# wangzy22/UniPre3D

Hardware: AMD Instinct MI355X
Metric: rendered_views_per_sec (higher is better)
Workload: dtype f32; 1 GPU; C2: render-loss hot path (activations + render fwd + loss + render bwd), object-level, P=128 Gaussians/object, 256x256, B=32/GPU x V=4 views = 128 renders/GPU/step; head output o ~ N(0,1) i.i.d. (SURVEY 8d primary regime); global_batch=32, parallelism=dp1, loss=focal_l2, autograd_entry=loss.backward()

## Files before the change

__graft_entry__.py:

```python
import os
import subprocess
import sys

ROOT = os.path.dirname(os.path.abspath(__file__))
if ROOT not in sys.path:
    sys.path.insert(0, ROOT)


def build() -> None:
    res = subprocess.run(["make", "-C", os.path.join(ROOT, "unipre3d_amd", "csrc"), "-j4"], capture_output=True, text=True)
    if res.returncode != 0:
        raise RuntimeError("HIP build failed:\n" + res.stdout[-3000:] + res.stderr[-3000:])
    import shutil
    csrc, var = os.path.join(ROOT, "unipre3d_amd", "csrc"), os.path.join(ROOT, "unipre3d_amd", "lib_general")
    res = subprocess.run(["make", "-C", csrc, "-j4", "LIBDIR=../lib_general", "EXTRA=-DU3D_FORCE_GENERAL", "../lib_general/libunipre3d_rasterizer.so"],
                         capture_output=True, text=True)
    if res.returncode != 0:
        raise RuntimeError("HIP build (test variant) failed:\n" + res.stdout[-3000:] + res.stderr[-3000:])
    shutil.copy2(os.path.join(ROOT, "unipre3d_amd", "lib", "_u3d_torch.so"), os.path.join(var, "_u3d_torch.so"))
    res = subprocess.run(["make", "-C", os.path.join(ROOT, "oracle")], capture_output=True, text=True)
    if res.returncode != 0:
        raise RuntimeError("oracle build failed:\n" + res.stdout[-3000:] + res.stderr[-3000:])
    import unipre3d_amd
    from unipre3d_amd import _lib
    lib = _lib.load()
    for name in _lib.EXPORTS:
        getattr(lib, name)
    from unipre3d_amd import rasterizer
    binding = rasterizer._C()
    for name in ("rasterize_view", "rasterize_batched", "render_loss_step", "unit_tensor", "abi_version"):
        getattr(binding, name)
    from unipre3d_amd import pointops
    po = pointops.load()
    for name in pointops.EXPORTS:
# ... 81 lines not shown
```

unipre3d_amd/csrc/u3d_common.h:

```cpp
#pragma once
#include <hip/hip_runtime.h>
#include <stdint.h>

#include "unipre3d_rasterizer.h"

#define U3D_TILE 16
#define U3D_BLOCK 256
#define U3D_WAVE 64
#define U3D_FLAG_INTERNAL_TRIAGE 0x40000000
#define U3D_TOUCHED_BIT 0x80000000u
#define U3D_TILE_PLAIN_BIT 0x80000000u
#define U3D_NACC 10
#define U3D_LDS_SORT_MAX 4096
static_assert(U3D_LDS_SORT_MAX == U3D_SPARSE_BWD_MIN_P, "the public header's sparse-backward threshold is this limit (the torch binding sizes its buffers by it)");
#ifndef U3D_RADIX_NT_SMALL
#define U3D_RADIX_NT_SMALL 1024
#define U3D_RADIX_IT_SMALL 2
#define U3D_RADIX_NT_LARGE 1024
#define U3D_RADIX_IT_LARGE 4
#endif
static inline int u3d_radix_tile(int P) { return P <= 65536 ? U3D_RADIX_NT_SMALL * U3D_RADIX_IT_SMALL : U3D_RADIX_NT_LARGE * U3D_RADIX_IT_LARGE; }
#define U3D_MSD_BINS_MAX 2048
static inline int u3d_msd_bins(int P) { return P <= 65536 ? 512 : (P <= 262144 ? 1024 : 2048); }
#define U3D_MSD_KEY_BASE 0x3E4CCCCDu

struct U3DBuffers {
  float* depth;
  float2* xy;
  float4* conic_op;
  float4* rgbd;
  uint2* rect;
  uint32_t* clamped;
  uint32_t* num_rendered;
  uint32_t* touched_words;
  uint2* touched_list;
  uint32_t* touched_count;
  uint32_t* sorted_id;
  uint2* sorted_rect;
  uint32_t* n_vis;
  uint32_t* sort_keys[2];
  uint32_t* sort_vals[2];
  uint2* sort_pairs;
  uint32_t* sort_hist;
  uint32_t* sort_over;
  float* final_T;
  uint32_t* n_contrib;
  uint32_t* tile_last;
};

struct U3DSpan {
  const int32_t* off;
  int P, vpi;
};
static inline U3DSpan u3d_span(const u3d_raster_desc& d) { return U3DSpan{d.total_P > 0 ? d.item_offsets : nullptr, d.P, d.views_per_item}; }
// ... 71 lines not shown
  float* qnorm; float* qdot; float* partial;
};
static inline size_t u3d_carve_fused(const u3d_raster_desc& d, void* base, U3DFused* f) {
  const size_t NV = (size_t)d.n_items * d.views_per_item;
  const size_t T = (size_t)((d.image_width + U3D_TILE - 1) / U3D_TILE) * ((d.image_height + U3D_TILE - 1) / U3D_TILE);
  const size_t a = (((size_t)d.n_items * 4 * sizeof(float)) + 255) & ~(size_t)255;
  if (f) {
    f->qnorm = (float*)base;
    f->qdot = (float*)((char*)base + a);
    f->partial = (float*)((char*)base + 2 * a);
  }
  return 2 * a + (((NV * T * sizeof(float)) + 255) & ~(size_t)255) + 256;
}

#define U3D_PART_BLOCKS 2
static inline int u3d_part_blocks(const u3d_raster_desc& d) { return d.P <= 256 ? 1 : U3D_PART_BLOCKS; }
#define U3D_PART_STRIDE (U3D_PART_BLOCKS * U3D_WAVE * 10)
static inline size_t u3d_align(size_t x) { return (x + 255) & ~(size_t)255; }

static inline U3DLayout u3d_carve(const u3d_raster_desc& d, void* geom, void* binning, void* image, U3DBuffers* b) {
  const size_t NV = (size_t)d.n_items * d.views_per_item, NG = (size_t)d.views_per_item * u3d_total_P(d);
  const size_t NP = NV * (size_t)d.image_height * d.image_width;
  U3DLayout L{};
  size_t o = 0;
  char* g = (char*)geom;
#define CARVE(base, field, type, count)        \
  do {                                         \
    if (b) b->field = (type*)(base + o);       \
    o += u3d_align(sizeof(type) * (count));    \
  } while (0)
  CARVE(g, depth, float, NG);
  CARVE(g, xy, float2, NG);
  CARVE(g, conic_op, float4, NG);
// ... 12 lines not shown
  CARVE(bn, sorted_rect, uint2, NG);
  CARVE(bn, n_vis, uint32_t, NV);
  if (d.P > U3D_LDS_SORT_MAX) {
    CARVE(bn, sort_keys[0], uint32_t, NG);
    CARVE(bn, sort_keys[1], uint32_t, NG);
    CARVE(bn, sort_vals[0], uint32_t, NG);
    CARVE(bn, sort_vals[1], uint32_t, NG);
    CARVE(bn, sort_pairs, uint2, NG);
    const size_t nblk = ((size_t)d.P + u3d_radix_tile(d.P) - 1) / u3d_radix_tile(d.P);
    CARVE(bn, sort_hist, uint32_t, NV * (size_t)u3d_msd_bins(d.P) * (nblk + 1));
    CARVE(bn, sort_over, uint32_t, NV * ((size_t)u3d_msd_bins(d.P) + 1));
  } else if (b) {
    b->sort_keys[0] = b->sort_keys[1] = b->sort_vals[0] = b->sort_vals[1] = b->sort_hist = b->sort_over = nullptr;
    b->sort_pairs = nullptr;
  }
  L.binning_bytes = o > 0 ? o : 256;
  o = 0;
  char* im = (char*)image;
  CARVE(im, final_T, float, NP);
  CARVE(im, n_contrib, uint32_t, NP);
  CARVE(im, tile_last, uint32_t, NV * (size_t)((d.image_width + U3D_TILE - 1) / U3D_TILE) * ((d.image_height + U3D_TILE - 1) / U3D_TILE));
  L.image_bytes = o > 0 ? o : 256;
#undef CARVE
  L.acc_bytes = u3d_align(sizeof(double) * U3D_NACC * (NG > 0 ? NG : 1));
  {
    const size_t Tn = (size_t)((d.image_width + U3D_TILE - 1) / U3D_TILE) * ((d.image_height + U3D_TILE - 1) / U3D_TILE);
    L.backward_bytes = L.acc_bytes + u3d_align(sizeof(float) * U3D_PART_STRIDE * (NV * Tn > 0 ? NV * Tn : 1)) +
                       u3d_align(sizeof(uint32_t) * (NV * Tn > 0 ? NV * Tn : 1));
  }
  L.fused_bytes = u3d_carve_fused(d, nullptr, nullptr);
// ... 107 lines not shown
```

unipre3d_amd/csrc/u3d_preprocess.hip:

```cpp
#include "u3d_common.h"

#pragma clang fp contract(off)

namespace {

constexpr float SH_C0 = 0.28209479177387814f;
constexpr float SH_C1 = 0.4886025119029199f;
__device__ constexpr float SH_C2[5] = {1.0925484305920792f, -1.0925484305920792f, 0.31539156525252005f,
                                       -1.0925484305920792f, 0.5462742152960396f};
__device__ constexpr float SH_C3[7] = {-0.5900435899266435f, 2.890611442640554f, -0.4570457994644658f,
                                       0.3731763325901154f,  -0.4570457994644658f, 1.445305721320277f,
                                       -0.5900435899266435f};

struct Cam {
  float V[16], Pm[16], pos[3];
};

__device__ __forceinline__ void load_cam(Cam& c, const float* __restrict__ view, const float* __restrict__ proj,
                                         const float* __restrict__ campos, int v) {
#pragma unroll
  for (int k = 0; k < 16; ++k) { c.V[k] = view[v * 16 + k]; c.Pm[k] = proj[v * 16 + k]; }
#pragma unroll
  for (int k = 0; k < 3; ++k) c.pos[k] = campos[v * 3 + k];
}
// ... 81 lines not shown
    for (int k = 0; k < 4; ++k) {
      g.raw_q[k] = g.q[k];
      g.qn[k] = fmaxf(src.act == 1 ? src.qnorm[item * 4 + k] : n4, 1e-6f);
      g.q[k] = g.q[k] / g.qn[k];
    }
  }
}

template <int D>
__global__ __launch_bounds__(U3D_BLOCK) void preprocess_fwd_kernel(
    U3DSpan span, int vpi, int vpt, int H, int W, float tanx, float tany, float mod, int flags, U3DSource src,
    const float* __restrict__ viewmatrix, const float* __restrict__ projmatrix, const float* __restrict__ campos,
    int32_t* __restrict__ radii, float* __restrict__ depth, float2* __restrict__ xy, float4* __restrict__ conic_op,
    float4* __restrict__ rgbd, uint2* __restrict__ rect, uint32_t* __restrict__ clamped,
    uint32_t* __restrict__ num_rendered, double* __restrict__ acc_zero, size_t NG, uint32_t* __restrict__ sorted_id,
    uint2* __restrict__ sorted_rect, uint32_t* __restrict__ n_vis, uint32_t* __restrict__ msd_total, int msd_bins,
    uint32_t* __restrict__ touched_words, uint8_t* __restrict__ visible, uint32_t* __restrict__ touched_count, uint32_t touched_count_init) {
  if (touched_count && blockIdx.x == 0 && blockIdx.y == 0 && blockIdx.z == 0 && threadIdx.x == 0) *touched_count = touched_count_init;
  if (msd_total && blockIdx.x == 0) {
    const int nv0 = blockIdx.z * vpt, nv1 = min(vpi, nv0 + vpt);
    for (int e = threadIdx.x; e < (nv1 - nv0) * msd_bins; e += U3D_BLOCK) msd_total[(size_t)(blockIdx.y * vpi + nv0) * msd_bins + e] = 0u;
  }
  __shared__ __attribute__((aligned(16))) unsigned long long s_keys[U3D_BLOCK];
  __shared__ uint2 s_rects[U3D_BLOCK];
  extern __shared__ __attribute__((aligned(16))) float s_rec[];
  constexpr int K = (D + 1) * (D + 1);
  const int item = blockIdx.y;
  int P;
  size_t gbase;
  u3d_set_span(span, item, P, gbase);
  const int i0 = blockIdx.x * U3D_BLOCK;
// ... 58 lines not shown
        const float* shr = lsrc.shs_rest + li * (size_t)lsrc.s_shs_rest;
#pragma unroll
        for (int k = 0; k < K * 3; ++k) shc[k] = k < 3 ? sh[k] : shr[k - 3];
      } else {
#pragma unroll
        for (int k = 0; k < K * 3; ++k) shc[k] = sh[k];
      }
    }
  }
  for (int vk = v0; vk < v1; ++vk) {
  const int view = item * vpi + vk;
  const size_t pbase = u3d_pair_base(span, vk, P, gbase);
  uint32_t touched = 0;
  unsigned long long sort_key = ~0ull;
  uint2 sort_rect = make_uint2(0u, 0u);
  if (i < P) {
    const size_t g = pbase + i;
    Cam cam;
    load_cam(cam, viewmatrix, projmatrix, campos, view);
    const float* p = gin.p;
    int radius = 0;
    float zv = cam.V[2] * p[0] + cam.V[6] * p[1] + cam.V[10] * p[2] + cam.V[14];
    float2 pix = make_float2(0.f, 0.f);
    float4 co = make_float4(0.f, 0.f, 0.f, 0.f), col = make_float4(0.f, 0.f, 0.f, 0.f);
    uint2 rc = make_uint2(0u, 0u);
    uint32_t cb = 0;
    if (zv > 0.2f) {
      float hom[4];
#pragma unroll
      for (int j = 0; j < 4; ++j) hom[j] = cam.Pm[j] * p[0] + cam.Pm[4 + j] * p[1] + cam.Pm[8 + j] * p[2] + cam.Pm[12 + j];
// ... 39 lines not shown
          col = make_float4(rgb[0], rgb[1], rgb[2], zv);
          rc = make_uint2((uint32_t)x0 | ((uint32_t)y0 << 16), (uint32_t)x1 | ((uint32_t)y1 << 16));
        }
      }
    }
    radii[g] = radius;
    if (visible) visible[g] = radius > 0 ? 1 : 0;
    depth[g] = radius > 0 ? zv : 0.f;
    xy[g] = pix;
    conic_op[g] = co;
    rgbd[g] = col;
    rect[g] = rc;
    clamped[g] = cb;
    if (radius > 0) sort_key = ((unsigned long long)__float_as_uint(zv) << 32) | (uint32_t)i;
    sort_rect = rc;
    if (acc_zero) {
#pragma unroll
      for (int k = 0; k < U3D_NACC; ++k) acc_zero[(size_t)k * NG + g] = 0.0;
    }
  }
  if (flags & U3D_FLAG_STATS) {
#pragma unroll
    for (int o = 32; o > 0; o >>= 1) touched += __shfl_xor(touched, o);
    if ((threadIdx.x & 63) == 0 && touched) atomicAdd(&num_rendered[view], touched);
  }
  if (sorted_id) {
    const int tid = threadIdx.x;
    __shared__ unsigned long long s_sorted[U3D_BLOCK];
    __syncthreads();
    const unsigned long long mine = sort_key != ~0ull ? sort_key : (0xFFFFFFFF00000000ull | (uint32_t)tid);
    s_keys[tid] = mine;
    s_rects[tid] = sort_rect;
    __syncthreads();
    {
      int rank = 0;
      const ulonglong2* k2 = reinterpret_cast<const ulonglong2*>(s_keys);
#pragma unroll 8
      for (int q = 0; q < U3D_BLOCK / 2; ++q) {
        const ulonglong2 two = k2[q];
        rank += (two.x < mine ? 1 : 0) + (two.y < mine ? 1 : 0);
      }
      s_sorted[rank] = mine;
    }
    __syncthreads();
    const unsigned long long kk = s_sorted[tid];
    const bool vis = (uint32_t)(kk >> 32) != 0xFFFFFFFFu;
    if (tid == 0 && !vis) n_vis[view] = 0;
    if (vis && (tid == U3D_BLOCK - 1 || (uint32_t)(s_sorted[tid + 1] >> 32) == 0xFFFFFFFFu)) n_vis[view] = (uint32_t)(tid + 1);
    if (tid < P) {
      const uint32_t id = vis ? (uint32_t)kk : 0u;
      sorted_id[pbase + tid] = id;
      sorted_rect[pbase + tid] = vis ? s_rects[id] : make_uint2(0u, 0u);
    }
  }
  }
}

// ... 444 lines not shown

void u3d_launch_preprocess_fwd(const u3d_raster_desc& d, const U3DBuffers& b, const U3DSource& src, const float* viewmatrix,
                               const float* projmatrix, const float* campos, int32_t* radii, double* acc_zero, hipStream_t s,
                               uint8_t* visible) {
  const bool fuse_sort = u3d_preprocess_sorts(d);
  const size_t NG = (size_t)d.views_per_item * u3d_total_P(d);
  const int vpt = (u3d_total_P(d) >= 65536) ? (d.views_per_item < 4 ? d.views_per_item : 4) : 1;
  const int chunks = (d.views_per_item + vpt - 1) / vpt;
  dim3 grid((d.P + U3D_BLOCK - 1) / U3D_BLOCK, d.n_items, chunks), block(U3D_BLOCK);
  const size_t lds = src.act != 0 ? (size_t)U3D_BLOCK * src.s_means * sizeof(float) : 0;
  const int D = src.shs ? d.sh_degree : 0;
#define LAUNCH(DEG)                                                                                                   \
  hipLaunchKernelGGL(preprocess_fwd_kernel<DEG>, grid, block, lds, s, u3d_span(d), d.views_per_item, vpt, d.image_height, \
                     d.image_width, d.tanfovx, d.tanfovy, d.scale_modifier, d.flags, src, viewmatrix, projmatrix, campos, \
                     radii, b.depth, b.xy, b.conic_op, b.rgbd, b.rect, b.clamped, b.num_rendered, acc_zero, NG,               \
                     fuse_sort ? b.sorted_id : nullptr, b.sorted_rect, b.n_vis, d.P > U3D_LDS_SORT_MAX ? b.sort_hist : nullptr, u3d_msd_bins(d.P), \
                     u3d_uses_touched_words(d) ? b.touched_words : nullptr, visible,                                      \
                     u3d_uses_touched_words(d) ? b.touched_count : nullptr,                                              \
                     u3d_sparse_bwd(d, src.act) ? 0u : U3D_TOUCHED_NOT_LISTED)
  switch (D) {
    case 0: LAUNCH(0); break;
    case 1: LAUNCH(1); break;
    case 2: LAUNCH(2); break;
    default: LAUNCH(3); break;
  }
#undef LAUNCH
}

void u3d_launch_preprocess_bwd(const u3d_raster_desc& d, const U3DBuffers& b, const U3DSource& src, const float* viewmatrix,
                               const float* projmatrix, const float* campos, const int32_t* radii, const double* acc,
                               const U3DGradSink& sink, hipStream_t s, double* acc_reset, const float* gscale, bool sparse) {
// ... 35 lines not shown
```

unipre3d_amd/csrc/u3d_render.hip:

```cpp
#include "u3d_common.h"
#if defined(U3D_LPT_EXPERIMENT) || defined(U3D_TIMELINE)
#include <algorithm>
#include <cstdio>
#include <vector>
#endif

namespace {

constexpr float LOG2E = 1.4426950408889634f;
constexpr float ALPHA_MIN = 1.0f / 255.0f;
constexpr float T_STOP = 0.0001f;
#ifndef U3D_FWD_HOIST
#define U3D_FWD_HOIST 1
#endif

__device__ __forceinline__ bool rect_hits(const uint2 r, int tx, int ty) {
  const int x0 = r.x & 0xffffu, y0 = r.x >> 16, x1 = r.y & 0xffffu, y1 = r.y >> 16;
  return tx >= x0 && tx < x1 && ty >= y0 && ty < y1;
}

struct LossCtx {
  int kind;
  float w_bg, w_non, b0, b1, b2, t0, t1, t2;
};
// ... 65 lines not shown
  return s < 1 ? 1 : (s > 32 ? 32 : s);
}
constexpr int TILE_WAVES = 1;

struct TileLds {
  float4* P0;
  float4* P1;
  float2* P2;
  float* D;
  float (*acc)[10];
  float* S;
  int sstride;
};
struct TileGeom {
  const uint32_t* sorted_id; const uint2* sorted_rect; const float2* xy; const float4* conic_op; const float4* rgbd;
  size_t vbase; int tx, ty;
  int rect_indirect;
  uint32_t* touched;
  uint32_t* tw;
  size_t gbase;
  uint2* tlist;
  uint32_t* tcount;
  uint32_t item;
};

template <bool DEPTH>
__device__ __forceinline__ lanemask_t tile_stage(const TileLds& L, const TileGeom& G, int lane, int b, uint32_t limit, bool& plain) {
  const uint32_t s = (uint32_t)b * U3D_WAVE + (uint32_t)lane;
  bool hit = false, ok = true;
  if (s < limit) hit = rect_hits(G.sorted_rect[G.vbase + (G.rect_indirect ? G.sorted_id[G.vbase + s] : s)], G.tx, G.ty);
  const lanemask_t bal = __ballot(hit);
  if (hit) {
    const uint32_t o = (uint32_t)__popcll(bal & ((1ull << lane) - 1ull));
    const size_t g = G.vbase + G.sorted_id[G.vbase + s];
    const float2 m = G.xy[g];
    const float4 co = G.conic_op[g];
    const float4 cd = G.rgbd[g];
    const float a1 = (-0.5f * LOG2E) * co.x, b1 = -LOG2E * co.y, c1 = (-0.5f * LOG2E) * co.z;
    L.P0[o] = make_float4(m.x, m.y, a1, b1);
    L.P1[o] = make_float4(c1, co.w, cd.x, cd.y);
    L.P2[o] = make_float2(cd.z, __uint_as_float(s + 1u));
    if (DEPTH) L.D[o] = 1.0f / cd.w;
    L.S[o * L.sstride] = __builtin_amdgcn_exp2f(a1 + a1);
    ok = a1 <= 0.f && a1 >= -2.5f && c1 <= 0.f && b1 * b1 <= (4.f * (1.f - 1e-5f)) * (a1 * c1) && co.w <= 0.98f && fabsf(m.x) < 1e30f && fabsf(m.y) < 1e30f;
// ... 16 lines not shown
  araw[1] = araw[0] * r;
  r *= s2;
  araw[2] = araw[1] * r;
  r *= s2;
  araw[3] = araw[2] * r;
}

struct TileFwd {
  float Tr[4], C0[4], C1[4], C2[4], Dv[4];
  uint32_t stop_pos[4];
  uint32_t wlast;
  int staged;
  lanemask_t staged_bal;
};

template <bool DEPTH, bool PLAIN>
__device__ __forceinline__ bool tile_forward(const TileLds& L, const TileGeom& G, int lane, uint32_t nv, float pyf,
                                             const float (&pxf)[4], const bool (&inside)[4], TileFwd& F) {
  float amin[4];
#pragma unroll
  for (int k = 0; k < 4; ++k) {
    F.Tr[k] = 1.f; F.C0[k] = F.C1[k] = F.C2[k] = F.Dv[k] = 0.f;
    amin[k] = inside[k] ? ALPHA_MIN : 2.f;
    F.stop_pos[k] = inside[k] ? 0xffffffffu : 0u;
  }
  F.wlast = 0; F.staged = -1; F.staged_bal = 0ull;
  int jlast = 0, blast = -1;
  bool wave_done = false;
  const int nbf = (int)((nv + U3D_WAVE - 1) / U3D_WAVE);
  for (int b = 0; b < nbf && !wave_done; ++b) {
    bool plain;
    const lanemask_t bal = tile_stage<DEPTH>(L, G, lane, b, nv, plain);
    if (PLAIN && !plain) return false;
    F.staged = b; F.staged_bal = bal;
    const int total = __popcll(bal);
    for (int j = 0; j < total; ++j) {
      const float4 A = L.P0[j];
      const float4 Q = L.P1[j];
      const float2 R = L.P2[j];
      const float invd = DEPTH ? L.D[j] : 0.f;
      const float dy = A.y - pyf;
      const float bdy = A.w * dy, cdy2 = (Q.x * dy) * dy;
      lanemask_t contrib = 0ull, m_stop[4];
      [[maybe_unused]] lanemask_t stopped = 0ull;
      float ar[4];
      if (PLAIN) alpha_run(A.x, A.z, bdy, cdy2, Q.y, L.S[j * L.sstride], pxf[0], ar);
#if U3D_FWD_HOIST
// ... 101 lines not shown
template <bool HAS_INVD, int PB , bool PLAIN >
__device__ __forceinline__ void tile_backward(const TileLds& L, const TileGeom& G, int lane, uint32_t wmax, int staged,
                                              lanemask_t staged_bal, float pyf, const float (&pxf)[4],
                                              const uint32_t (&lim)[4], float (&Tr)[4], float (&Rk)[4],
                                              const float (&dp0)[4], const float (&dp1)[4], const float (&dp2)[4],
                                              const float (&dinv)[4], float half_w, float half_h, size_t NG,
                                              double* __restrict__ acc, float* __restrict__ pt, uint32_t* __restrict__ pcnt) {
  constexpr int NK = HAS_INVD ? U3D_NACC : U3D_NACC - 1;
  const int bank = (lane >> 2) & 3;
  const bool writer = (lane & 3) == 0 && lane < 16;
  typedef __attribute__((address_space(3))) float lds_float;
  const uint32_t acc_lane = (uint32_t)(uintptr_t)(lds_float*)&L.acc[0][0] + 4u * (uint32_t)bank;
  const int nb = (int)((wmax + U3D_WAVE - 1) / U3D_WAVE);
  for (int b = nb - 1; b >= 0; --b) {
    lanemask_t bal = staged_bal;
    if (b != staged) { bool plain; bal = tile_stage<HAS_INVD>(L, G, lane, b, wmax, plain); staged = b; staged_bal = bal; }
    const uint32_t lm = wmax - (uint32_t)b * U3D_WAVE;
    const int total = lm >= U3D_WAVE ? __popcll(bal) : __popcll(bal & ((1ull << lm) - 1ull));
    for (int j = total - 1; j >= 0; --j) {
      const float4 A = L.P0[j];
      const float4 Q = L.P1[j];
      const float2 R = L.P2[j];
      const float invd = HAS_INVD ? L.D[j] : 0.f;
      const uint32_t pos = __float_as_uint(R.y);
      const float dy = A.y - pyf;
      const float bdy = A.w * dy, cdy2 = (Q.x * dy) * dy;
      float dx[4], ae[4], ar[4];
      lanemask_t any = 0ull;
      if (PLAIN) alpha_run(A.x, A.z, bdy, cdy2, Q.y, L.S[j * L.sstride], pxf[0], ar);
#pragma unroll
      for (int k = 0; k < 4; ++k) {
// ... 206 lines not shown
  const int px0 = tx * U3D_TILE + 4 * (lane & 3);                                                       \
  const float pyf = (float)py;                                                                          \
  const size_t npix = (size_t)H * W;                                                                    \
  [[maybe_unused]] const size_t pid0 = (size_t)view * npix + (size_t)py * W + px0;  \
  const size_t cid0 = (size_t)view * 3 * npix + (size_t)py * W + px0;             \
  const bool vec = (W & 3) == 0;                                                                        \
  float pxf[4];                                                                                         \
  bool inside[4];                                                                                       \
  _Pragma("unroll") for (int k = 0; k < 4; ++k) {                                                       \
    pxf[k] = (float)(px0 + k);                                                                          \
    inside[k] = px0 + k < W && py < H;                                                                  \
  }                                                                                                     \
  int Pv_;         \
  size_t vb_;                                                                                            \
  u3d_view_span(span, view, Pv_, vb_);                                                                   \
  const TileGeom G{sorted_id, sorted_rect, xy, conic_op, rgbd, vb_, tx, ty, rect_indirect, touched, touched_words, touched_words ? u3d_view_gbase(span, view) : 0, \
                   tlist, tcount, (uint32_t)(view / span.vpi)}

template <bool DEPTH>
__global__ __launch_bounds__(TILE_WAVES * U3D_WAVE) void render_fwd_wave_kernel(
    U3DSpan span, int H, int W, int tiles_x, int T, uint32_t ntiles_total, uint32_t tile_magic, const uint32_t* __restrict__ sorted_id,
    const uint2* __restrict__ sorted_rect, int rect_indirect, const uint32_t* __restrict__ n_vis, const float2* __restrict__ xy,
    const float4* __restrict__ conic_op, const float4* __restrict__ rgbd, const float* __restrict__ bg,
    float* __restrict__ out_color, float* __restrict__ out_invdepth, float* __restrict__ final_T,
    uint32_t* __restrict__ n_contrib, uint32_t* __restrict__ tile_last, U3DLoss loss) {
  uint32_t* const touched = nullptr;
  uint32_t* const touched_words = nullptr;
  uint2* const tlist = nullptr;
  uint32_t* const tcount = nullptr;
  __shared__ float4 sP0[TILE_WAVES][U3D_WAVE], sP1[TILE_WAVES][U3D_WAVE];
  __shared__ float2 sP2[TILE_WAVES][U3D_WAVE];
  __shared__ float sD[TILE_WAVES][DEPTH ? U3D_WAVE : 1];
  __shared__ float sS[TILE_WAVES][U3D_WAVE];
  U3D_TILE_PROLOGUE(TILE_WAVES);
  const TileLds L{sP0[wave], sP1[wave], sP2[wave], sD[wave], nullptr, sS[wave], 1};
  TileFwd F;
  const uint32_t nv = n_vis[view];
  const bool plain = tile_forward<DEPTH, true>(L, G, lane, nv, pyf, pxf, inside, F);
  if (!plain) tile_forward<DEPTH, false>(L, G, lane, nv, pyf, pxf, inside, F);

  float o0[4], o1[4], o2[4], lim[4];
#pragma unroll
  for (int k = 0; k < 4; ++k) {
    o0[k] = fmaf(F.Tr[k], bg[0], F.C0[k]); o1[k] = fmaf(F.Tr[k], bg[1], F.C1[k]); o2[k] = fmaf(F.Tr[k], bg[2], F.C2[k]);
    lim[k] = __uint_as_float(F.stop_pos[k]);
  }
  store4(final_T + pid0, vec, inside, F.Tr);
  store4(reinterpret_cast<float*>(n_contrib) + pid0, vec, inside, lim);
  store4(out_color + cid0, vec, inside, o0);
  store4(out_color + cid0 + npix, vec, inside, o1);
  store4(out_color + cid0 + 2 * npix, vec, inside, o2);
  if (DEPTH) store4(out_invdepth + pid0, vec, inside, F.Dv);
  if (lane == 0) tile_last[lid] = F.wlast | (plain ? U3D_TILE_PLAIN_BIT : 0u);
  if (loss.kind != 0) {
// ... 9 lines not shown
    if (lane == 0) loss.partial[lid] = e;
  }
}

#ifndef U3D_BWD_OCC_PIN
#define U3D_BWD_OCC_PIN 7
#endif
#if U3D_BWD_OCC_PIN
#define U3D_BWD_OCCUPANCY __attribute__((amdgpu_waves_per_eu((PB == 1 && !HAS_INVD) ? U3D_BWD_OCC_PIN : 1, (PB == 1 && !HAS_INVD) ? U3D_BWD_OCC_PIN : 10)))
#else
#define U3D_BWD_OCCUPANCY
#endif
template <bool HAS_INVD, int PB>
__global__ __launch_bounds__(TILE_WAVES * U3D_WAVE) U3D_BWD_OCCUPANCY void render_bwd_wave_kernel(
    U3DSpan span, int H, int W, int tiles_x, int T, uint32_t ntiles_total, uint32_t tile_magic, size_t NG,
    const uint32_t* __restrict__ sorted_id, const uint2* __restrict__ sorted_rect, int rect_indirect, const float2* __restrict__ xy,
    const float4* __restrict__ conic_op, const float4* __restrict__ rgbd, const float* __restrict__ bg,
    const float* __restrict__ dL_dcolor, const float* __restrict__ dL_dinvdepth, const float* __restrict__ final_T,
    const uint32_t* __restrict__ n_contrib, const uint32_t* __restrict__ tile_last, double* __restrict__ acc,
    float* __restrict__ part, const float* __restrict__ out_color, uint32_t* __restrict__ touched, uint32_t* __restrict__ touched_words,
    U3DLoss loss) {
  uint2* const tlist = nullptr;
  uint32_t* const tcount = nullptr;
  __shared__ float4 sP0[TILE_WAVES][U3D_WAVE], sP1[TILE_WAVES][U3D_WAVE];
  __shared__ float2 sP2[TILE_WAVES][U3D_WAVE];
  __shared__ float sD[TILE_WAVES][HAS_INVD ? U3D_WAVE : 1];
  __shared__ __attribute__((aligned(8))) float sAcc[TILE_WAVES][U3D_WAVE][10];
  __shared__ float sS[TILE_WAVES][HAS_INVD ? U3D_WAVE : 1];
  U3D_TILE_PROLOGUE(TILE_WAVES);
  const TileLds L{sP0[wave], sP1[wave], sP2[wave], sD[wave], sAcc[wave], HAS_INVD ? sS[wave] : &sAcc[wave][0][9], HAS_INVD ? 1 : 10};
#pragma unroll
  for (int k = 0; k < 5; ++k) reinterpret_cast<float2*>(&sAcc[wave][lane][0])[k] = make_float2(0.f, 0.f);

  float Tr[4], Rk[4], dp0[4], dp1[4], dp2[4], dinv[4], limf[4];
  uint32_t lim[4];
  load4(final_T + pid0, vec, inside, Tr);
  load4(reinterpret_cast<const float*>(n_contrib) + pid0, vec, inside, limf);
// ... 34 lines not shown
  }
  const uint32_t tl = tile_last[lid];
  if (tl & U3D_TILE_PLAIN_BIT)
    tile_backward<HAS_INVD, PB, true>(L, G, lane, tl & ~U3D_TILE_PLAIN_BIT, -1, 0ull, pyf, pxf, lim, Tr, Rk, dp0, dp1, dp2, dinv, 0.5f * (float)W,
                          0.5f * (float)H, NG, acc, part + (size_t)lid * (PB * U3D_WAVE * 10),
                          reinterpret_cast<uint32_t*>(part + (size_t)ntiles_total * BWD_PART_STRIDE) + lid);
  else
    tile_backward<HAS_INVD, PB, false>(L, G, lane, tl, -1, 0ull, pyf, pxf, lim, Tr, Rk, dp0, dp1, dp2, dinv, 0.5f * (float)W,
                          0.5f * (float)H, NG, acc, part + (size_t)lid * (PB * U3D_WAVE * 10),
                          reinterpret_cast<uint32_t*>(part + (size_t)ntiles_total * BWD_PART_STRIDE) + lid);
}

template <int PB>
__global__ __launch_bounds__(TILE_WAVES * U3D_WAVE) U3D_FULL_OCCUPANCY void render_fb_wave_kernel(
    U3DSpan span, int H, int W, int tiles_x, int T, uint32_t ntiles_total, uint32_t tile_magic, size_t NG,
    const uint32_t* __restrict__ sorted_id, const uint2* __restrict__ sorted_rect, int rect_indirect, const uint32_t* __restrict__ n_vis,
    const float2* __restrict__ xy, const float4* __restrict__ conic_op, const float4* __restrict__ rgbd,
    const float* __restrict__ bg, float* __restrict__ out_color, double* __restrict__ acc, float* __restrict__ part,
    uint32_t* __restrict__ touched, uint32_t* __restrict__ touched_words, uint2* __restrict__ tlist, uint32_t* __restrict__ tcount,
    U3DLoss loss) {
  __shared__ float4 sP0[TILE_WAVES][U3D_WAVE], sP1[TILE_WAVES][U3D_WAVE];
  __shared__ float2 sP2[TILE_WAVES][U3D_WAVE];
  __shared__ __attribute__((aligned(8))) float sAcc[TILE_WAVES][U3D_WAVE][10];
#ifdef U3D_TIMELINE
  const uint64_t tl_t0 = __builtin_amdgcn_s_memrealtime(), tl_c0 = __builtin_amdgcn_s_memtime();
#endif
#ifdef U3D_PRIO_FWD
  __builtin_amdgcn_s_setprio(U3D_PRIO_FWD);
#endif
  U3D_TILE_PROLOGUE(TILE_WAVES);
  const TileLds L{sP0[wave], sP1[wave], sP2[wave], nullptr, sAcc[wave], &sAcc[wave][0][9], 10};
#pragma unroll
  for (int k = 0; k < 5; ++k) reinterpret_cast<float2*>(&sAcc[wave][lane][0])[k] = make_float2(0.f, 0.f);
  TileFwd F;
  const uint32_t nv = n_vis[view];
  const bool plain = tile_forward<false, true>(L, G, lane, nv, pyf, pxf, inside, F);
  if (!plain) tile_forward<false, false>(L, G, lane, nv, pyf, pxf, inside, F);
#ifdef U3D_TIMELINE
  const uint64_t tl_t1 = __builtin_amdgcn_s_memrealtime();
#endif

  float dp0[4], dp1[4], dp2[4], dinv[4], Rk[4], o0[4], o1[4], o2[4], g0[4], g1[4], g2[4];
  float e = 0.f;
#pragma unroll
  for (int k = 0; k < 4; ++k) {
    o0[k] = fmaf(F.Tr[k], bg[0], F.C0[k]); o1[k] = fmaf(F.Tr[k], bg[1], F.C1[k]); o2[k] = fmaf(F.Tr[k], bg[2], F.C2[k]);
  }
  load4(loss.gt + cid0, vec, inside, g0);
  load4(loss.gt + cid0 + npix, vec, inside, g1);
  load4(loss.gt + cid0 + 2 * npix, vec, inside, g2);
  if (out_color) {
    store4(out_color + cid0, vec, inside, o0);
// ... 285 lines not shown
static inline TileGrid tile_grid(const u3d_raster_desc& d, int tiles_x, int T) {
  const uint32_t NV = (uint32_t)(d.n_items * d.views_per_item);
  const uint32_t gy = NV < 65535u ? NV : 65535u, gz = (NV + gy - 1u) / gy;
  uint32_t magic = 0u;
  if (tiles_x > 1 && (uint64_t)T * (uint64_t)tiles_x < (1ull << 32)) magic = (uint32_t)(((1ull << 32) + (uint64_t)tiles_x - 1ull) / (uint64_t)tiles_x);
  return TileGrid{dim3((uint32_t)T, gy, gz), magic};
}

void u3d_launch_render_fwd(const u3d_raster_desc& d, const U3DBuffers& b, const float* bg, float* out_color,
                           float* out_invdepth, const U3DLoss& loss, hipStream_t s) {
  const int tiles_x = (d.image_width + U3D_TILE - 1) / U3D_TILE, tiles_y = (d.image_height + U3D_TILE - 1) / U3D_TILE;
  const int T = tiles_x * tiles_y;
  const uint32_t ntiles = (uint32_t)(d.n_items * d.views_per_item * T);
  if (ntiles == 0) return;
  const TileGrid tg = tile_grid(d, tiles_x, T);
  auto* kern = out_invdepth ? render_fwd_wave_kernel<true> : render_fwd_wave_kernel<false>;
  hipLaunchKernelGGL(kern, tg.grid, dim3(TILE_WAVES * U3D_WAVE), 0, s, u3d_span(d), d.image_height, d.image_width,
                     tiles_x, T, ntiles, tg.magic, b.sorted_id, u3d_rect_indirect(d) ? b.rect : b.sorted_rect, u3d_rect_indirect(d), b.n_vis, b.xy, b.conic_op, b.rgbd, bg, out_color,
                     out_invdepth, b.final_T, b.n_contrib, b.tile_last, loss);
}

void u3d_launch_render_fb(const u3d_raster_desc& d, const U3DBuffers& b, const float* bg, float* out_color,
                          const U3DLoss& loss, double* acc, float* part, float* loss_out, hipStream_t s,
                          float* zero_fill, size_t zero_floats, bool list_touched) {
  const int tiles_x = (d.image_width + U3D_TILE - 1) / U3D_TILE, tiles_y = (d.image_height + U3D_TILE - 1) / U3D_TILE;
  const int T = tiles_x * tiles_y;
  const uint32_t ntiles = (uint32_t)(d.n_items * d.views_per_item * T);
  const size_t NG = (size_t)d.views_per_item * u3d_total_P(d);
  if (ntiles == 0 || NG == 0) return;
  const TileGrid tg = tile_grid(d, tiles_x, T);
  uint32_t* tw = u3d_uses_touched_words(d) ? b.touched_words : nullptr;
  uint2* tl = (list_touched && tw) ? b.touched_list : nullptr;
  uint32_t* tc = (list_touched && tw) ? b.touched_count : nullptr;
// ... 52 lines not shown
      }
      if (launches == at + 6) {
        (void)hipStreamSynchronize(s);
        std::vector<uint4> h(2 * (size_t)ntiles);
        (void)hipMemcpy(h.data(), d_tl, 2 * sizeof(uint4) * ntiles, hipMemcpyDeviceToHost);
        uint4* nul = nullptr;
        (void)hipMemcpyToSymbol(HIP_SYMBOL(g_timeline), &nul, sizeof(nul));
        if (FILE* f = fopen(out, "wb")) { fwrite(h.data(), sizeof(uint4), 2 * (size_t)ntiles, f); fclose(f); }
        fprintf(stderr, "[timeline] %u tiles of launch %d -> %s\n", ntiles, at + 5, out);
      }
    }
  }
#endif
  if (u3d_part_blocks(d) == 1)
    hipLaunchKernelGGL(render_fb_wave_kernel<1>, tg.grid, dim3(TILE_WAVES * U3D_WAVE), 0, s, u3d_span(d), d.image_height, d.image_width,
                       tiles_x, T, ntiles, tg.magic, NG, b.sorted_id, u3d_rect_indirect(d) ? b.rect : b.sorted_rect, u3d_rect_indirect(d), b.n_vis, b.xy, b.conic_op, b.rgbd, bg, out_color,
                       acc, part, b.clamped, tw, tl, tc, loss);
  else
    hipLaunchKernelGGL(render_fb_wave_kernel<U3D_PART_BLOCKS>, tg.grid, dim3(TILE_WAVES * U3D_WAVE), 0, s, u3d_span(d), d.image_height,
                       d.image_width, tiles_x, T, ntiles, tg.magic, NG, b.sorted_id, u3d_rect_indirect(d) ? b.rect : b.sorted_rect, u3d_rect_indirect(d), b.n_vis, b.xy, b.conic_op, b.rgbd, bg,
                       out_color, acc, part, b.clamped, tw, tl, tc, loss);
  const int nsplit = bwd_reduce_split(T, d.n_items * d.views_per_item);
  const int NVi = d.n_items * d.views_per_item;
  if (u3d_part_blocks(d) == 1) {
    hipLaunchKernelGGL(bwd_reduce1_kernel, dim3(NVi, nsplit + 1), dim3(REDUCE_THREADS), 0, s,
                       u3d_span(d), T, U3D_NACC - 1, nsplit, NG, 0.5f * (float)d.image_width, 0.5f * (float)d.image_height, b.sorted_id, b.conic_op, part,
                       reinterpret_cast<const uint32_t*>(part + (size_t)ntiles * BWD_PART_STRIDE), acc, b.clamped, tw, (int)ntiles, loss.partial,
                       loss.inv_count, loss_out);
  } else {
    int zrows = 0;
    if (zero_fill && zero_floats > 0) {
      const size_t want = (zero_floats * sizeof(float) + 65535) / 65536;
      zrows = (int)((want < 256 ? want : 256) + (size_t)NVi - 1) / NVi;
      if (zrows < 1) zrows = 1;
    }
// ... 5 lines not shown
}

void u3d_launch_render_bwd(const u3d_raster_desc& d, const U3DBuffers& b, const float* bg, const float* dL_dcolor,
                           const float* dL_dinvdepth, const float* out_color, const U3DLoss& loss, double* acc,
                           float* part, hipStream_t s) {
  const int tiles_x = (d.image_width + U3D_TILE - 1) / U3D_TILE, tiles_y = (d.image_height + U3D_TILE - 1) / U3D_TILE;
  const int T = tiles_x * tiles_y;
  const uint32_t ntiles = (uint32_t)(d.n_items * d.views_per_item * T);
  const size_t NG = (size_t)d.views_per_item * u3d_total_P(d);
  if (ntiles == 0 || NG == 0) return;
  const TileGrid tg = tile_grid(d, tiles_x, T);
  const bool invd = dL_dinvdepth && loss.kind == 0;
  uint32_t* tw = u3d_uses_touched_words(d) ? b.touched_words : nullptr;
#define LAUNCH(INVD, PBV)                                                                                                   \
  hipLaunchKernelGGL((render_bwd_wave_kernel<INVD, PBV>), tg.grid, dim3(TILE_WAVES * U3D_WAVE), 0, s, u3d_span(d), d.image_height, \
                     d.image_width, tiles_x, T, ntiles, tg.magic, NG, b.sorted_id, u3d_rect_indirect(d) ? b.rect : b.sorted_rect, u3d_rect_indirect(d), b.xy, b.conic_op, b.rgbd, bg,    \
                     dL_dcolor, dL_dinvdepth, b.final_T, b.n_contrib, b.tile_last, acc, part, out_color, b.clamped, tw, loss)
  if (u3d_part_blocks(d) == 1) { if (invd) LAUNCH(true, 1); else LAUNCH(false, 1); }
  else { if (invd) LAUNCH(true, U3D_PART_BLOCKS); else LAUNCH(false, U3D_PART_BLOCKS); }
#undef LAUNCH
  const int nsplit = bwd_reduce_split(T, d.n_items * d.views_per_item);
  if (u3d_part_blocks(d) == 1)
    hipLaunchKernelGGL(bwd_reduce1_kernel, dim3(d.n_items * d.views_per_item, nsplit), dim3(REDUCE_THREADS), 0, s,
                       u3d_span(d), T, invd ? U3D_NACC : U3D_NACC - 1, nsplit, NG, 0.5f * (float)d.image_width, 0.5f * (float)d.image_height, b.sorted_id,
                       b.conic_op, part, reinterpret_cast<const uint32_t*>(part + (size_t)ntiles * BWD_PART_STRIDE), acc, b.clamped, tw, 0, nullptr, 0.f,
                       nullptr);
  else
    hipLaunchKernelGGL(bwd_reduce_kernel<U3D_PART_BLOCKS>, dim3(d.n_items * d.views_per_item, nsplit), dim3(REDUCE_THREADS), 0, s,
                       u3d_span(d), T, invd ? U3D_NACC : U3D_NACC - 1, nsplit, NG, 0.5f * (float)d.image_width, 0.5f * (float)d.image_height, b.sorted_id,
                       b.conic_op, part, reinterpret_cast<const uint32_t*>(part + (size_t)ntiles * BWD_PART_STRIDE), acc, b.clamped, tw, 0, nullptr, 0.f,
                       nullptr, (uint2*)nullptr, (uint32_t*)nullptr, (float*)nullptr, (size_t)0);
// ... 2 lines not shown
```

Before: 658,200 views/s.

## Stage depth-sorted per-Gaussian records in preprocess for streamed tile loading

When P fits one block, the fused preprocess/sort kernel now writes each visible Gaussian's precomputed rasterization parameters (position, log2e-scaled conic terms, opacity, color, signed inverse depth, rect) into three contiguous float4 planes in sorted order. The render forward, fused forward-backward and backward tile loops then read these records with plain streaming loads instead of the sorted_id indirection and gather from xy, conic_op, rgbd and rect. This removes dependent gathers and per-tile recomputation in the hot raster loops. In exchange the preprocess kernel does extra global writes and uses more binning memory. A gather-only variant library is also built for comparison.

```diff
diff --git a/__graft_entry__.py b/__graft_entry__.py
--- a/__graft_entry__.py
+++ b/__graft_entry__.py
@@ -18,6 +18,12 @@
     if res.returncode != 0:
         raise RuntimeError("HIP build (test variant) failed:\n" + res.stdout[-3000:] + res.stderr[-3000:])
     shutil.copy2(os.path.join(ROOT, "unipre3d_amd", "lib", "_u3d_torch.so"), os.path.join(var, "_u3d_torch.so"))
+    gat = os.path.join(ROOT, "unipre3d_amd", "lib_gather")
+    res = subprocess.run(["make", "-C", csrc, "-j4", "LIBDIR=../lib_gather", "EXTRA=-DU3D_STAGE_GATHER", "../lib_gather/libunipre3d_rasterizer.so"],
+                         capture_output=True, text=True)
+    if res.returncode != 0:
+        raise RuntimeError("HIP build (gather variant) failed:\n" + res.stdout[-3000:] + res.stderr[-3000:])
+    shutil.copy2(os.path.join(ROOT, "unipre3d_amd", "lib", "_u3d_torch.so"), os.path.join(gat, "_u3d_torch.so"))
     res = subprocess.run(["make", "-C", os.path.join(ROOT, "oracle")], capture_output=True, text=True)
     if res.returncode != 0:
         raise RuntimeError("oracle build failed:\n" + res.stdout[-3000:] + res.stderr[-3000:])
diff --git a/unipre3d_amd/csrc/u3d_common.h b/unipre3d_amd/csrc/u3d_common.h
--- a/unipre3d_amd/csrc/u3d_common.h
+++ b/unipre3d_amd/csrc/u3d_common.h
@@ -38,6 +38,7 @@
   uint32_t* sorted_id;
   uint2* sorted_rect;
   uint32_t* n_vis;
+  float4* stage;
   uint32_t* sort_keys[2];
   uint32_t* sort_vals[2];
   uint2* sort_pairs;
@@ -139,9 +140,22 @@
 }
 
 #define U3D_PART_BLOCKS 2
-static inline int u3d_part_blocks(const u3d_raster_desc& d) { return d.P <= 256 ? 1 : U3D_PART_BLOCKS; }
+static inline bool u3d_has_stage(const u3d_raster_desc& d) { return d.P <= U3D_BLOCK; }
+static inline int u3d_part_blocks(const u3d_raster_desc& d) { return u3d_has_stage(d) ? 1 : U3D_PART_BLOCKS; }
 #define U3D_PART_STRIDE (U3D_PART_BLOCKS * U3D_WAVE * 10)
 static inline size_t u3d_align(size_t x) { return (x + 255) & ~(size_t)255; }
+
+#define U3D_STAGE_PLANES 3
+#define U3D_STAGE_LOG2E 1.4426950408889634f
+#ifdef __HIPCC__
+struct U3DStaged { float a1, b1, c1; bool ok; };
+__device__ __forceinline__ U3DStaged u3d_stage_values(const float2 m, const float4 co) {
+  U3DStaged v;
+  v.a1 = (-0.5f * U3D_STAGE_LOG2E) * co.x; v.b1 = -U3D_STAGE_LOG2E * co.y; v.c1 = (-0.5f * U3D_STAGE_LOG2E) * co.z;
+  v.ok = v.a1 <= 0.f && v.a1 >= -2.5f && v.c1 <= 0.f && v.b1 * v.b1 <= (4.f * (1.f - 1e-5f)) * (v.a1 * v.c1) && co.w <= 0.98f && fabsf(m.x) < 1e30f && fabsf(m.y) < 1e30f;
+  return v;
+}
+#endif
 
 static inline U3DLayout u3d_carve(const u3d_raster_desc& d, void* geom, void* binning, void* image, U3DBuffers* b) {
   const size_t NV = (size_t)d.n_items * d.views_per_item, NG = (size_t)d.views_per_item * u3d_total_P(d);
@@ -184,6 +198,8 @@
     b->sort_keys[0] = b->sort_keys[1] = b->sort_vals[0] = b->sort_vals[1] = b->sort_hist = b->sort_over = nullptr;
     b->sort_pairs = nullptr;
   }
+  if (u3d_has_stage(d)) CARVE(bn, stage, float4, U3D_STAGE_PLANES * NG);
+  else if (b) b->stage = nullptr;
   L.binning_bytes = o > 0 ? o : 256;
   o = 0;
   char* im = (char*)image;
diff --git a/unipre3d_amd/csrc/u3d_preprocess.hip b/unipre3d_amd/csrc/u3d_preprocess.hip
--- a/unipre3d_amd/csrc/u3d_preprocess.hip
+++ b/unipre3d_amd/csrc/u3d_preprocess.hip
@@ -119,7 +119,7 @@
     int32_t* __restrict__ radii, float* __restrict__ depth, float2* __restrict__ xy, float4* __restrict__ conic_op,
     float4* __restrict__ rgbd, uint2* __restrict__ rect, uint32_t* __restrict__ clamped,
     uint32_t* __restrict__ num_rendered, double* __restrict__ acc_zero, size_t NG, uint32_t* __restrict__ sorted_id,
-    uint2* __restrict__ sorted_rect, uint32_t* __restrict__ n_vis, uint32_t* __restrict__ msd_total, int msd_bins,
+    uint2* __restrict__ sorted_rect, float4* __restrict__ stage, uint32_t* __restrict__ n_vis, uint32_t* __restrict__ msd_total, int msd_bins,
     uint32_t* __restrict__ touched_words, uint8_t* __restrict__ visible, uint32_t* __restrict__ touched_count, uint32_t touched_count_init) {
   if (touched_count && blockIdx.x == 0 && blockIdx.y == 0 && blockIdx.z == 0 && threadIdx.x == 0) *touched_count = touched_count_init;
   if (msd_total && blockIdx.x == 0) {
@@ -208,6 +208,8 @@
   uint32_t touched = 0;
   unsigned long long sort_key = ~0ull;
   uint2 sort_rect = make_uint2(0u, 0u);
+  float2 st_xy = make_float2(0.f, 0.f);
+  float4 st_co = make_float4(0.f, 0.f, 0.f, 0.f), st_col = make_float4(0.f, 0.f, 0.f, 0.f);
   if (i < P) {
     const size_t g = pbase + i;
     Cam cam;
@@ -277,6 +279,7 @@
     clamped[g] = cb;
     if (radius > 0) sort_key = ((unsigned long long)__float_as_uint(zv) << 32) | (uint32_t)i;
     sort_rect = rc;
+    st_xy = pix; st_co = co; st_col = col;
     if (acc_zero) {
 #pragma unroll
       for (int k = 0; k < U3D_NACC; ++k) acc_zero[(size_t)k * NG + g] = 0.0;
@@ -304,6 +307,14 @@
         rank += (two.x < mine ? 1 : 0) + (two.y < mine ? 1 : 0);
       }
       s_sorted[rank] = mine;
+      if (stage && sort_key != ~0ull) {
+        const U3DStaged v = u3d_stage_values(st_xy, st_co);
+        const float invd = 1.0f / st_col.w;
+        float4* rec = stage + pbase + rank;
+        rec[0] = make_float4(st_xy.x, st_xy.y, v.a1, v.b1);
+        rec[NG] = make_float4(v.c1, st_co.w, st_col.x, st_col.y);
+        rec[2 * NG] = make_float4(st_col.z, v.ok ? invd : -invd, __uint_as_float(sort_rect.x), __uint_as_float(sort_rect.y));
+      }
     }
     __syncthreads();
     const unsigned long long kk = s_sorted[tid];
@@ -778,7 +789,7 @@
   hipLaunchKernelGGL(preprocess_fwd_kernel<DEG>, grid, block, lds, s, u3d_span(d), d.views_per_item, vpt, d.image_height, \
                      d.image_width, d.tanfovx, d.tanfovy, d.scale_modifier, d.flags, src, viewmatrix, projmatrix, campos, \
                      radii, b.depth, b.xy, b.conic_op, b.rgbd, b.rect, b.clamped, b.num_rendered, acc_zero, NG,               \
-                     fuse_sort ? b.sorted_id : nullptr, b.sorted_rect, b.n_vis, d.P > U3D_LDS_SORT_MAX ? b.sort_hist : nullptr, u3d_msd_bins(d.P), \
+                     fuse_sort ? b.sorted_id : nullptr, b.sorted_rect, fuse_sort ? b.stage : nullptr, b.n_vis, d.P > U3D_LDS_SORT_MAX ? b.sort_hist : nullptr, u3d_msd_bins(d.P), \
                      u3d_uses_touched_words(d) ? b.touched_words : nullptr, visible,                                      \
                      u3d_uses_touched_words(d) ? b.touched_count : nullptr,                                              \
                      u3d_sparse_bwd(d, src.act) ? 0u : U3D_TOUCHED_NOT_LISTED)
diff --git a/unipre3d_amd/csrc/u3d_render.hip b/unipre3d_amd/csrc/u3d_render.hip
--- a/unipre3d_amd/csrc/u3d_render.hip
+++ b/unipre3d_amd/csrc/u3d_render.hip
@@ -103,6 +103,8 @@
 };
 struct TileGeom {
   const uint32_t* sorted_id; const uint2* sorted_rect; const float2* xy; const float4* conic_op; const float4* rgbd;
+  const float4* stage;
+  size_t nstage;
   size_t vbase; int tx, ty;
   int rect_indirect;
   uint32_t* touched;
@@ -113,10 +115,40 @@
   uint32_t item;
 };
 
-template <bool DEPTH>
+#ifdef U3D_STAGE_GATHER
+#define U3D_STREAM(x) false
+#else
+#define U3D_STREAM(x) (x)
+#endif
+template <bool DEPTH, bool STREAM>
 __device__ __forceinline__ lanemask_t tile_stage(const TileLds& L, const TileGeom& G, int lane, int b, uint32_t limit, bool& plain) {
   const uint32_t s = (uint32_t)b * U3D_WAVE + (uint32_t)lane;
   bool hit = false, ok = true;
+  if (STREAM) {
+    float4 q0, q1, q2;
+    if (s < limit) {
+      const float4* rec = G.stage + G.vbase + s;
+      q0 = rec[0]; q1 = rec[G.nstage]; q2 = rec[2 * G.nstage];
+      hit = rect_hits(make_uint2(__float_as_uint(q2.z), __float_as_uint(q2.w)), G.tx, G.ty);
+    }
+    const lanemask_t bal = __ballot(hit);
+    if (hit) {
+      const uint32_t o = (uint32_t)__popcll(bal & ((1ull << lane) - 1ull));
+      L.P0[o] = q0;
+      L.P1[o] = q1;
+      L.P2[o] = make_float2(q2.x, __uint_as_float(s + 1u));
+      if (DEPTH) L.D[o] = __uint_as_float(__float_as_uint(q2.y) & 0x7fffffffu);
+      L.S[o * L.sstride] = __builtin_amdgcn_exp2f(q0.z + q0.z);
+      ok = (int)__float_as_uint(q2.y) >= 0;
+    }
+#ifdef U3D_FORCE_GENERAL
+    ok = false;
+#endif
+    plain = __ballot(!ok) == 0ull;
+    __builtin_amdgcn_fence(__ATOMIC_RELEASE, "wavefront");
+    __builtin_amdgcn_wave_barrier();
+    return bal;
+  }
   if (s < limit) hit = rect_hits(G.sorted_rect[G.vbase + (G.rect_indirect ? G.sorted_id[G.vbase + s] : s)], G.tx, G.ty);
   const lanemask_t bal = __ballot(hit);
   if (hit) {
@@ -163,7 +195,7 @@
   lanemask_t staged_bal;
 };
 
-template <bool DEPTH, bool PLAIN>
+template <bool DEPTH, bool PLAIN, bool STREAM>
 __device__ __forceinline__ bool tile_forward(const TileLds& L, const TileGeom& G, int lane, uint32_t nv, float pyf,
                                              const float (&pxf)[4], const bool (&inside)[4], TileFwd& F) {
   float amin[4];
@@ -179,7 +211,7 @@
   const int nbf = (int)((nv + U3D_WAVE - 1) / U3D_WAVE);
   for (int b = 0; b < nbf && !wave_done; ++b) {
     bool plain;
-    const lanemask_t bal = tile_stage<DEPTH>(L, G, lane, b, nv, plain);
+    const lanemask_t bal = tile_stage<DEPTH, STREAM>(L, G, lane, b, nv, plain);
     if (PLAIN && !plain) return false;
     F.staged = b; F.staged_bal = bal;
     const int total = __popcll(bal);
@@ -311,7 +343,7 @@
   const int nb = (int)((wmax + U3D_WAVE - 1) / U3D_WAVE);
   for (int b = nb - 1; b >= 0; --b) {
     lanemask_t bal = staged_bal;
-    if (b != staged) { bool plain; bal = tile_stage<HAS_INVD>(L, G, lane, b, wmax, plain); staged = b; staged_bal = bal; }
+    if (b != staged) { bool plain; bal = tile_stage<HAS_INVD, U3D_STREAM(PB == 1)>(L, G, lane, b, wmax, plain); staged = b; staged_bal = bal; }
     const uint32_t lm = wmax - (uint32_t)b * U3D_WAVE;
     const int total = lm >= U3D_WAVE ? __popcll(bal) : __popcll(bal & ((1ull << lm) - 1ull));
     for (int j = total - 1; j >= 0; --j) {
@@ -548,13 +580,13 @@
   int Pv_;         \
   size_t vb_;                                                                                            \
   u3d_view_span(span, view, Pv_, vb_);                                                                   \
-  const TileGeom G{sorted_id, sorted_rect, xy, conic_op, rgbd, vb_, tx, ty, rect_indirect, touched, touched_words, touched_words ? u3d_view_gbase(span, view) : 0, \
+  const TileGeom G{sorted_id, sorted_rect, xy, conic_op, rgbd, stage, nstage, vb_, tx, ty, rect_indirect, touched, touched_words, touched_words ? u3d_view_gbase(span, view) : 0, \
                    tlist, tcount, (uint32_t)(view / span.vpi)}
 
-template <bool DEPTH>
+template <bool DEPTH, bool STREAM>
 __global__ __launch_bounds__(TILE_WAVES * U3D_WAVE) void render_fwd_wave_kernel(
     U3DSpan span, int H, int W, int tiles_x, int T, uint32_t ntiles_total, uint32_t tile_magic, const uint32_t* __restrict__ sorted_id,
-    const uint2* __restrict__ sorted_rect, int rect_indirect, const uint32_t* __restrict__ n_vis, const float2* __restrict__ xy,
+    const uint2* __restrict__ sorted_rect, const float4* __restrict__ stage, size_t nstage, int rect_indirect, const uint32_t* __restrict__ n_vis, const float2* __restrict__ xy,
     const float4* __restrict__ conic_op, const float4* __restrict__ rgbd, const float* __restrict__ bg,
     float* __restrict__ out_color, float* __restrict__ out_invdepth, float* __restrict__ final_T,
     uint32_t* __restrict__ n_contrib, uint32_t* __restrict__ tile_last, U3DLoss loss) {
@@ -570,8 +602,8 @@
   const TileLds L{sP0[wave], sP1[wave], sP2[wave], sD[wave], nullptr, sS[wave], 1};
   TileFwd F;
   const uint32_t nv = n_vis[view];
-  const bool plain = tile_forward<DEPTH, true>(L, G, lane, nv, pyf, pxf, inside, F);
-  if (!plain) tile_forward<DEPTH, false>(L, G, lane, nv, pyf, pxf, inside, F);
+  const bool plain = tile_forward<DEPTH, true, STREAM>(L, G, lane, nv, pyf, pxf, inside, F);
+  if (!plain) tile_forward<DEPTH, false, STREAM>(L, G, lane, nv, pyf, pxf, inside, F);
 
   float o0[4], o1[4], o2[4], lim[4];
 #pragma unroll
@@ -611,13 +643,14 @@
 template <bool HAS_INVD, int PB>
 __global__ __launch_bounds__(TILE_WAVES * U3D_WAVE) U3D_BWD_OCCUPANCY void render_bwd_wave_kernel(
     U3DSpan span, int H, int W, int tiles_x, int T, uint32_t ntiles_total, uint32_t tile_magic, size_t NG,
-    const uint32_t* __restrict__ sorted_id, const uint2* __restrict__ sorted_rect, int rect_indirect, const float2* __restrict__ xy,
-    const float4* __restrict__ conic_op, const float4* __restrict__ rgbd, const float* __restrict__ bg,
+    const uint32_t* __restrict__ sorted_id, const uint2* __restrict__ sorted_rect, const float4* __restrict__ stage, int rect_indirect,
+    const float2* __restrict__ xy, const float4* __restrict__ conic_op, const float4* __restrict__ rgbd, const float* __restrict__ bg,
     const float* __restrict__ dL_dcolor, const float* __restrict__ dL_dinvdepth, const float* __restrict__ final_T,
     const uint32_t* __restrict__ n_contrib, const uint32_t* __restrict__ tile_last, double* __restrict__ acc,
     float* __restrict__ part, const float* __restrict__ out_color, uint32_t* __restrict__ touched, uint32_t* __restrict__ touched_words,
     U3DLoss loss) {
   uint2* const tlist = nullptr;
+  const size_t nstage = NG;
   uint32_t* const tcount = nullptr;
   __shared__ float4 sP0[TILE_WAVES][U3D_WAVE], sP1[TILE_WAVES][U3D_WAVE];
   __shared__ float2 sP2[TILE_WAVES][U3D_WAVE];
@@ -682,13 +715,14 @@
 template <int PB>
 __global__ __launch_bounds__(TILE_WAVES * U3D_WAVE) U3D_FULL_OCCUPANCY void render_fb_wave_kernel(
     U3DSpan span, int H, int W, int tiles_x, int T, uint32_t ntiles_total, uint32_t tile_magic, size_t NG,
-    const uint32_t* __restrict__ sorted_id, const uint2* __restrict__ sorted_rect, int rect_indirect, const uint32_t* __restrict__ n_vis,
-    const float2* __restrict__ xy, const float4* __restrict__ conic_op, const float4* __restrict__ rgbd,
+    const uint32_t* __restrict__ sorted_id, const uint2* __restrict__ sorted_rect, const float4* __restrict__ stage, int rect_indirect,
+    const uint32_t* __restrict__ n_vis, const float2* __restrict__ xy, const float4* __restrict__ conic_op, const float4* __restrict__ rgbd,
     const float* __restrict__ bg, float* __restrict__ out_color, double* __restrict__ acc, float* __restrict__ part,
     uint32_t* __restrict__ touched, uint32_t* __restrict__ touched_words, uint2* __restrict__ tlist, uint32_t* __restrict__ tcount,
     U3DLoss loss) {
   __shared__ float4 sP0[TILE_WAVES][U3D_WAVE], sP1[TILE_WAVES][U3D_WAVE];
   __shared__ float2 sP2[TILE_WAVES][U3D_WAVE];
+  const size_t nstage = NG;
   __shared__ __attribute__((aligned(8))) float sAcc[TILE_WAVES][U3D_WAVE][10];
 #ifdef U3D_TIMELINE
   const uint64_t tl_t0 = __builtin_amdgcn_s_memrealtime(), tl_c0 = __builtin_amdgcn_s_memtime();
@@ -702,8 +736,8 @@
   for (int k = 0; k < 5; ++k) reinterpret_cast<float2*>(&sAcc[wave][lane][0])[k] = make_float2(0.f, 0.f);
   TileFwd F;
   const uint32_t nv = n_vis[view];
-  const bool plain = tile_forward<false, true>(L, G, lane, nv, pyf, pxf, inside, F);
-  if (!plain) tile_forward<false, false>(L, G, lane, nv, pyf, pxf, inside, F);
+  const bool plain = tile_forward<false, true, U3D_STREAM(PB == 1)>(L, G, lane, nv, pyf, pxf, inside, F);
+  if (!plain) tile_forward<false, false, U3D_STREAM(PB == 1)>(L, G, lane, nv, pyf, pxf, inside, F);
 #ifdef U3D_TIMELINE
   const uint64_t tl_t1 = __builtin_amdgcn_s_memrealtime();
 #endif
@@ -1019,9 +1053,12 @@
   const uint32_t ntiles = (uint32_t)(d.n_items * d.views_per_item * T);
   if (ntiles == 0) return;
   const TileGrid tg = tile_grid(d, tiles_x, T);
-  auto* kern = out_invdepth ? render_fwd_wave_kernel<true> : render_fwd_wave_kernel<false>;
+  const bool stream = U3D_STREAM(u3d_has_stage(d));
+  auto* kern = stream ? (out_invdepth ? render_fwd_wave_kernel<true, true> : render_fwd_wave_kernel<false, true>)
+                      : (out_invdepth ? render_fwd_wave_kernel<true, false> : render_fwd_wave_kernel<false, false>);
   hipLaunchKernelGGL(kern, tg.grid, dim3(TILE_WAVES * U3D_WAVE), 0, s, u3d_span(d), d.image_height, d.image_width,
-                     tiles_x, T, ntiles, tg.magic, b.sorted_id, u3d_rect_indirect(d) ? b.rect : b.sorted_rect, u3d_rect_indirect(d), b.n_vis, b.xy, b.conic_op, b.rgbd, bg, out_color,
+                     tiles_x, T, ntiles, tg.magic, b.sorted_id, u3d_rect_indirect(d) ? b.rect : b.sorted_rect, b.stage,
+                     (size_t)d.views_per_item * u3d_total_P(d), u3d_rect_indirect(d), b.n_vis, b.xy, b.conic_op, b.rgbd, bg, out_color,
                      out_invdepth, b.final_T, b.n_contrib, b.tile_last, loss);
 }
 
@@ -1104,11 +1141,11 @@
 #endif
   if (u3d_part_blocks(d) == 1)
     hipLaunchKernelGGL(render_fb_wave_kernel<1>, tg.grid, dim3(TILE_WAVES * U3D_WAVE), 0, s, u3d_span(d), d.image_height, d.image_width,
-                       tiles_x, T, ntiles, tg.magic, NG, b.sorted_id, u3d_rect_indirect(d) ? b.rect : b.sorted_rect, u3d_rect_indirect(d), b.n_vis, b.xy, b.conic_op, b.rgbd, bg, out_color,
+                       tiles_x, T, ntiles, tg.magic, NG, b.sorted_id, u3d_rect_indirect(d) ? b.rect : b.sorted_rect, b.stage, u3d_rect_indirect(d), b.n_vis, b.xy, b.conic_op, b.rgbd, bg, out_color,
                        acc, part, b.clamped, tw, tl, tc, loss);
   else
     hipLaunchKernelGGL(render_fb_wave_kernel<U3D_PART_BLOCKS>, tg.grid, dim3(TILE_WAVES * U3D_WAVE), 0, s, u3d_span(d), d.image_height,
-                       d.image_width, tiles_x, T, ntiles, tg.magic, NG, b.sorted_id, u3d_rect_indirect(d) ? b.rect : b.sorted_rect, u3d_rect_indirect(d), b.n_vis, b.xy, b.conic_op, b.rgbd, bg,
+                       d.image_width, tiles_x, T, ntiles, tg.magic, NG, b.sorted_id, u3d_rect_indirect(d) ? b.rect : b.sorted_rect, b.stage, u3d_rect_indirect(d), b.n_vis, b.xy, b.conic_op, b.rgbd, bg,
                        out_color, acc, part, b.clamped, tw, tl, tc, loss);
   const int nsplit = bwd_reduce_split(T, d.n_items * d.views_per_item);
   const int NVi = d.n_items * d.views_per_item;
@@ -1144,7 +1181,7 @@
   uint32_t* tw = u3d_uses_touched_words(d) ? b.touched_words : nullptr;
 #define LAUNCH(INVD, PBV)                                                                                                   \
   hipLaunchKernelGGL((render_bwd_wave_kernel<INVD, PBV>), tg.grid, dim3(TILE_WAVES * U3D_WAVE), 0, s, u3d_span(d), d.image_height, \
-                     d.image_width, tiles_x, T, ntiles, tg.magic, NG, b.sorted_id, u3d_rect_indirect(d) ? b.rect : b.sorted_rect, u3d_rect_indirect(d), b.xy, b.conic_op, b.rgbd, bg,    \
+                     d.image_width, tiles_x, T, ntiles, tg.magic, NG, b.sorted_id, u3d_rect_indirect(d) ? b.rect : b.sorted_rect, b.stage, u3d_rect_indirect(d), b.xy, b.conic_op, b.rgbd, bg,    \
                      dL_dcolor, dL_dinvdepth, b.final_T, b.n_contrib, b.tile_last, acc, part, out_color, b.clamped, tw, loss)
   if (u3d_part_blocks(d) == 1) { if (invd) LAUNCH(true, 1); else LAUNCH(false, 1); }
   else { if (invd) LAUNCH(true, U3D_PART_BLOCKS); else LAUNCH(false, U3D_PART_BLOCKS); }
```

Measured after the change: 659,000 views/s, median of 3. No clear change (+0.1%).
